# beecave-homelab/VibeVoice-ROCm

Measured on AMD Instinct MI355X. Metric: audio-sec/s, higher is better.
Workload: dtype bf16; 1 GPU; cfg2: VibeVoice-1.5B shapes, 1 speaker(s) x 203-frame voice prompt, 330-token prompt, 225 frames (30.0 s audio), CFG=2.0, 20 DPM-Solver++ steps, whole generate() incl. voice encode + prefill; global_batch=1, parallelism=replicas x1 (one dialogue per GPU), hipgraph=True

## Files before the change

### include/vv_hip.h

```cpp
#ifndef VV_HIP_H
#define VV_HIP_H

#include <stddef.h>
#include <stdint.h>

#ifdef __cplusplus
extern "C" {
#endif

typedef void* vv_stream_t;

enum { VV_F32 = 0, VV_BF16 = 1, VV_FP8 = 2  };
enum { VV_NF4 = 3 };
enum { VV_WQ_NF4 = 0x100 };
enum { VV_OK = 0, VV_E_ARG = -1, VV_E_HIP = -2, VV_E_UNSUPPORTED = -3 };
enum { VV_PRO_NONE = 0, VV_PRO_RMSNORM = 1, VV_PRO_SILU = 2 };
enum { VV_ACT_NONE = 0, VV_ACT_GELU = 1, VV_ACT_SWIGLU = 2 };
enum { VV_LIN_X_BF16 = 1, VV_LIN_OUT_BF16 = 2, VV_LIN_W_REUSED = 4, VV_LIN_W_FRAG = 8 };

const char* vv_last_error(void);
int vv_abi_version(void);
int vv_tune(const char* key, int value);
int vv_init(void);

// ... 185 lines not shown
int vv_encoder_forward(const vv_convnet* net, const float* wav, int64_t T, float* feat, void* ws, vv_stream_t stream);
int vv_convnet_reset(const vv_convnet* net, vv_stream_t stream);

typedef struct vv_connector { int wdt, din, hidden; const void* fc1; const float* b1; const float* norm_w; const void* fc2; const float* b2; } vv_connector;
int vv_connector_forward(const vv_connector* c, const float* x, int R, float* out, int accumulate, float* ws, vv_stream_t stream);
int vv_connector_pair(const vv_connector* ac, const vv_connector* sem, const float* latent, const float* semfeat, float* out, int64_t ldo,
                      int rows_out, float* ws, vv_stream_t stream);

int vv_graph_begin(vv_stream_t stream);
int vv_graph_end(vv_stream_t stream, void** graph_exec_out);
int vv_graph_launch(void* graph_exec, vv_stream_t stream);
int vv_graph_destroy(void* graph_exec);

typedef struct vv_prof_entry { int m, n, k, dual, wdt, count; double total_ms; } vv_prof_entry;
int vv_prof_begin(int max_records);
int vv_prof_end(vv_prof_entry* out, int max_out, int* n_out);

typedef struct vv_nf4_src {
  const uint8_t* packed;
  const void* absmax;
  const float* quant_map;
  const float* nested_absmax;
  const float* nested_map;
  float nested_offset;
  int nested_blocksize;
  int n, k, blocksize;
} vv_nf4_src;
int vv_nf4_import(const vv_nf4_src* src, void* w, int64_t ldw, int row0, int rows_total, void* cq, float* cs, vv_stream_t stream);

#define VV_CONV_HOT_GEMV 0
#define VV_CONV_HOT_ROW 1
typedef struct vv_conv_hot_shape { const char* name; int kind, m, n, k, bias, gate, res; } vv_conv_hot_shape;
int vv_conv_hot_shapes(vv_conv_hot_shape* out, int cap);

size_t vv_sizeof(const char* struct_name);

#ifdef __cplusplus
}
#endif
#endif
```

### vibevoice_rocm_amd/_lib.py

```python
from __future__ import annotations

import ctypes as C
import os

_HERE = os.path.dirname(os.path.abspath(__file__))
LIB_PATH = os.path.join(_HERE, "libvv_hip.so")

VV_F32, VV_BF16, VV_FP8, VV_NF4 = 0, 1, 2, 3
VV_WQ_NF4 = 0x100
PRO_NONE, PRO_RMSNORM, PRO_SILU = 0, 1, 2
ACT_NONE, ACT_GELU, ACT_SWIGLU = 0, 1, 2
LIN_X_BF16, LIN_OUT_BF16, LIN_W_REUSED, LIN_W_FRAG = 1, 2, 4, 8
VV_MAX_STAGES = 8
KVQ_DERIVE_SCALES = 1

vp = C.c_void_p
i64 = C.c_int64


class W8(C.Structure):
    _fields_ = [("q", vp), ("scale", vp)]


class LinArgs(C.Structure):
# ... 103 lines not shown
    "vv_add_rows_silu_bf16": (C.c_int, [vp, i64, vp, i64, vp, C.c_int, C.c_int, C.c_int, vp]),
    "vv_dpm_proj": (C.c_int, [vp, i64, C.c_float, C.POINTER(DpmCoef), vp, vp, vp, vp, vp, C.c_int, C.c_int, C.c_int, vp, i64, C.c_int, vp, vp]),
    "vv_embed_row": (C.c_int, [vp, C.c_int, i64, vp, vp, vp]),
    "vv_gather_rows": (C.c_int, [vp, C.c_int, i64, C.POINTER(C.c_int), C.c_int, vp, vp]),
    "vv_argmax_ids": (C.c_int, [vp, C.c_int, vp, vp, vp, vp]),
    "vv_cast_rows_bf16": (C.c_int, [vp, i64, C.c_int, C.c_int, C.c_int, vp, C.c_float, vp, i64, vp]),
    "vv_copy_rows": (C.c_int, [vp, i64, vp, i64, C.c_int, C.c_int, vp]),
    "vv_dpm_step": (C.c_int, [vp, i64, C.c_int, C.c_int, C.c_float, C.c_float, C.c_float, C.c_float, C.c_float,
                              C.c_float, C.c_int, vp, vp, vp]),
    "vv_advance_lens": (C.c_int, [vp, vp, C.c_int, C.c_int, vp, vp]),
    "vv_llm_ws_bytes": (C.c_size_t, [C.POINTER(Llm), C.c_int]),
    "vv_llm_forward": (C.c_int, [C.POINTER(Llm), C.POINTER(KV), vp, i64, C.c_int, vp, vp, vp, i64, vp, vp]),
    "vv_llm_tail": (C.c_int, [C.POINTER(Llm), vp, i64, C.c_int, vp, i64, vp, C.c_int, vp, vp, vp, vp, vp, C.c_int, C.c_int, vp, vp]),
    "vv_llm_tail_batch": (C.c_int, [C.POINTER(Llm), vp, i64, C.c_int, vp, i64, vp, C.c_int, vp, vp, vp, vp, vp, C.c_int, C.c_int, vp, vp, vp]),
    "vv_head_ws_bytes": (C.c_size_t, [C.POINTER(Head), C.c_int]),
    "vv_head_ws_bytes_batch": (C.c_size_t, [C.POINTER(Head), C.c_int, C.c_int]),
    "vv_head_sample_batch": (C.c_int, [C.POINTER(Head), vp, i64, vp, i64, vp, C.POINTER(DpmCoef), C.c_int, C.c_float, vp, i64, C.c_int, vp, vp]),
    "vv_head_ws_bytes_batch_sde": (C.c_size_t, [C.POINTER(Head), C.c_int, C.c_int]),
    "vv_head_sample_batch_sde": (C.c_int, [C.POINTER(Head), vp, i64, vp, i64, vp, C.POINTER(DpmCoef), C.c_int, C.c_float, vp, i64, C.c_int, vp, vp, i64, vp]),
    "vv_head_sample": (C.c_int, [C.POINTER(Head), vp, i64, vp, vp, C.POINTER(DpmCoef), C.c_int, C.c_float, vp, vp, vp, vp]),
    "vv_head_forward": (C.c_int, [C.POINTER(Head), vp, vp, vp, C.c_int, vp, vp, vp]),
    "vv_convnet_ws_bytes": (C.c_size_t, [C.POINTER(ConvNet), i64, C.c_int]),
    "vv_decoder_forward": (C.c_int, [C.POINTER(ConvNet), vp, C.c_int, C.c_float, C.c_float, vp, vp, vp]),
    "vv_encoder_forward": (C.c_int, [C.POINTER(ConvNet), vp, i64, vp, vp, vp]),
    "vv_convnet_reset": (C.c_int, [C.POINTER(ConvNet), vp]),
    "vv_connector_forward": (C.c_int, [C.POINTER(Connector), vp, C.c_int, vp, C.c_int, vp, vp]),
    "vv_connector_pair": (C.c_int, [C.POINTER(Connector), C.POINTER(Connector), vp, vp, vp, i64, C.c_int, vp, vp]),
    "vv_graph_begin": (C.c_int, [vp]),
    "vv_graph_end": (C.c_int, [vp, C.POINTER(vp)]),
    "vv_graph_launch": (C.c_int, [vp, vp]),
    "vv_graph_destroy": (C.c_int, [vp]),
    "vv_nf4_import": (C.c_int, [C.POINTER(Nf4Src), vp, i64, C.c_int, C.c_int, vp, vp, vp]),
    "vv_conv_hot_shapes": (C.c_int, [vp, C.c_int]),
    "vv_sizeof": (C.c_size_t, [C.c_char_p]),
    "vv_prof_begin": (C.c_int, [C.c_int]),
    "vv_prof_end": (C.c_int, [C.POINTER(ProfEntry), C.c_int, C.POINTER(C.c_int)]),
}


class VVError(RuntimeError):
    pass


_lib = None


def load():
    global _lib
    if _lib is not None:
        return _lib
    import torch
    if not os.path.exists(LIB_PATH):
        raise VVError(f"{LIB_PATH} is missing: build the HIP extension first (python -m vibevoice_rocm_amd.build). "
                      "The MI355X kernels are the only compute path of this package.")
    lib = C.CDLL(LIB_PATH)
    for name, (res, args) in PROTOTYPES.items():
        fn = getattr(lib, name)
        fn.restype = res
        fn.argtypes = args
    for cname, cls in _STRUCTS.items():
        n = lib.vv_sizeof(cname.encode())
        if n != C.sizeof(cls):
            raise VVError(f"ABI mismatch for {cname}: C side {n} bytes, ctypes mirror {C.sizeof(cls)} bytes")
    _lib = lib
    return lib

# ... 9 lines not shown
```

### vibevoice_rocm_amd/csrc/vv_common.h

```cpp
#ifndef VV_COMMON_H
#define VV_COMMON_H
#include <hip/hip_runtime.h>
#include <stdarg.h>
#include <stdint.h>
#include "vv_hip.h"

int vv_set_error(int code, const char* fmt, ...);

#define VV_CHECK_LAUNCH(name)                                                                    \
  do {                                                                                           \
    hipError_t e_ = hipGetLastError();                                                           \
    if (e_ != hipSuccess) return vv_set_error(VV_E_HIP, "%s: %s", name, hipGetErrorString(e_));  \
  } while (0)

#define VV_TRY(expr)            \
  do {                          \
    int rc_ = (expr);           \
    if (rc_) return rc_;        \
  } while (0)

struct vv_kv_args {
  void* k; void* v;
  int kvdt, layers, rows, kv_heads, s_max, head_dim;
  void* vt;
  vv_kv_args(const vv_kv& a) : k(a.k), v(a.v), kvdt(a.kvdt), layers(a.layers), rows(a.rows), kv_heads(a.kv_heads), s_max(a.s_max), head_dim(a.head_dim), vt(a.vt) {}
};
struct vv_kv_args8 : vv_kv_args {
  const float* kscale; const float* vscale;
  vv_kv_args8(const vv_kv& a) : vv_kv_args(a), kscale(a.kscale), vscale(a.vscale) {}
};

int vv_launch_gemv_stream(const vv_lin_args& a, hipStream_t s);
struct vv_gemv_hot_shape { const char* name; int m, n, k, dual, pro, mod, bias, gate, res, act, flags; };
extern "C" int vv_gemv_hot_shapes(vv_gemv_hot_shape* out, int cap);
int vv_launch_gemv_hot(const vv_lin_args& a, hipStream_t s);
void vv_gemv_hot_set(int mask);
int vv_launch_conv_hot_gemv(const vv_lin_args& a, hipStream_t s);
int vv_launch_conv_hot_row(const vv_block& B, const float* x, float* y, float* hidden, float* hist_new, int C, float eps, hipStream_t s);
void vv_conv_hot_set(int mask);
int vv_launch_gemv_rows(const vv_lin_args& a, float* part, size_t part_floats, int* tickets, size_t n_tickets, hipStream_t s);
size_t vv_gemv_rows_part_floats(int n, int dual);
size_t vv_gemv_rows_tickets(int n);
int vv_gemv_rows_init();
void vv_gemv_rows_set(int on, int blocks, int pers);
int vv_linear_ws(const vv_lin_args* a, const void* f1, const void* f2, float* part, size_t part_floats, int* tickets, size_t n_tickets,
                 vv_stream_t stream, const vv_w8* q1 = nullptr, const vv_w8* q2 = nullptr);
int vv_launch_mfma_gemm(const vv_lin_args& a, hipStream_t s);
int vv_mfma_gemm_init();
int vv_launch_attn_decode(const float* qkv, int64_t ld_qkv, int R, int heads, const vv_kv* kv, int layer, const float2* rope, const int* lens, float* out,
                          int64_t ldo, float* part, int* tickets, int nsplit, int part_cap, hipStream_t s);
int vv_attn_decode_ws(const float* qkv, int64_t ld_qkv, int R, int heads, const vv_kv* kv, int layer, const float* rope_table, const int* lens, float* out,
                      int64_t ldo, float* part, int* tickets, int nsplit, int part_cap, vv_stream_t stream);
int vv_launch_kv_quantize(const vv_kv* src, const vv_kv* dst, int src_row, int dst_row, int len, int flags, hipStream_t s);
int vv_launch_attn_prefill(const float* qkv, int64_t ld_qkv, int R, int heads, const vv_kv* kv, int layer, const int* lens, const int* cache_rows,
                           float* out, int64_t ldo, hipStream_t s);
int vv_head_init_fused(const vv_head* h, const float* noise, float* Xs, float* Ms, float* h0, int64_t ldh, hipStream_t s);
bool vv_head_boundary_supported(const vv_head* h);
int vv_head_boundary_fused(const vv_head* h, const float* hrows, int64_t ldh, const float* shift, const float* scale, int64_t ld_mod, float cfg,
                           const vv_dpm_coef* k, float* Xs, float* Ms, float* h_out, int64_t ldh_out, float* latent_out, hipStream_t s);
int vv_head_boundary_batch(const vv_head* h, const float* hrows, int64_t ldh, const float* shift, const float* scale, int64_t ld_mod, float cfg,
                           const vv_dpm_coef* k, float* Xs, float* Ms, int64_t state_stride, float* h_out, int64_t ldh_out, float* latent_out,
                           int64_t latent_stride, int B, hipStream_t s,
                           const float* nx = nullptr, int64_t nx_stride = 0);
int vv_head_sde_proj_fused(const vv_head* h, const float* sde_noise, int64_t ld_sde, int n_steps, int B, float* NX, hipStream_t s);
int vv_fused_init();
int vv_head_pre_fused(const vv_head* h, const float* cond2, int64_t ld_cond, const float* temb, int n_steps, void* c_bf16, const float* noise,
                      float* Xs, float* Ms, float* h0, int64_t ldh, hipStream_t s);
int vv_launch_connector_pair(const vv_connector* ac, const vv_connector* sem, const float* latent, const float* semfeat, float* out, int64_t ldo, int rows_out,
                             float* ws, hipStream_t s);
int vv_head_modulations_fused(const vv_head* h, const void* c_bf16, int rows, float* const* mod, float* modf, hipStream_t s);
struct vv_conv_ctx_item { float* pad; float* state; int ctx, T, C; const float* dw_w; float* hs; int affine; float scale, bias; };
// ... 59 lines not shown
```

### vibevoice_rocm_amd/csrc/vv_conv_hot.hip

```cpp
#include <hip/hip_runtime.h>
#include <hip/hip_bf16.h>
#include <stdint.h>

#include "vv_hip.h"
#include "vv_common.h"

namespace {

typedef unsigned short bf16_t;
typedef unsigned int u32x4 __attribute__((ext_vector_type(4)));
typedef float vf2 __attribute__((ext_vector_type(2)));
typedef __bf16 bf16x8 __attribute__((ext_vector_type(8)));
typedef float f32x16 __attribute__((ext_vector_type(16)));

__device__ __forceinline__ void unpack8(const u32x4 v, float (&o)[8]) {
  o[0] = __uint_as_float(v.x << 16); o[1] = __uint_as_float(v.x & 0xffff0000u);
  o[2] = __uint_as_float(v.y << 16); o[3] = __uint_as_float(v.y & 0xffff0000u);
  o[4] = __uint_as_float(v.z << 16); o[5] = __uint_as_float(v.z & 0xffff0000u);
  o[6] = __uint_as_float(v.w << 16); o[7] = __uint_as_float(v.w & 0xffff0000u);
}

template <bool NT>
__device__ __forceinline__ u32x4 ldw(const bf16_t* p) {
  const u32x4* q = reinterpret_cast<const u32x4*>(p);
  if constexpr (NT) return __builtin_nontemporal_load(q);
  else return *q;
}

__device__ __forceinline__ void fma_unit(const u32x4 wv, const float (&x)[8], vf2& p) {
  float w[8];
  unpack8(wv, w);
#pragma unroll
  for (int j = 0; j < 8; j += 2) p = __builtin_elementwise_fma(vf2{w[j], w[j + 1]}, vf2{x[j], x[j + 1]}, p);
}

__device__ __forceinline__ float gate_res(float v, float g, float r) {
#pragma clang fp contract(off)
  const float t = v * g;
  return t + r;
}

#define VV_FENCE4(v) asm volatile("" : "+v"((v).x), "+v"((v).y), "+v"((v).z), "+v"((v).w))

template <int N, int K, int NW, int R, bool GR>
__global__ __launch_bounds__(64 * NW) void conv_gemv_kernel(const vv_lin_args a) {
  constexpr int KU = K / (512 * NW);
// ... 163 lines not shown
      uint2 p;
      p.x = pack2(yv[j][0] * rstd2 * fw[j][0], yv[j][1] * rstd2 * fw[j][1]);
      p.y = pack2(yv[j][2] * rstd2 * fw[j][2], yv[j][3] * rstd2 * fw[j][3]);
      *reinterpret_cast<uint2*>(xh + c0[j]) = p;
      if (c0[j] >= ys0 && c0[j] < ys0 + C / ROW_WG) st4(y + c0[j], yv[j]);
    }
  }
  __syncthreads();
  f32x16 acc;
#pragma unroll
  for (int i = 0; i < 16; ++i) acc[i] = 0.f;
  {
    const bf16_t* xf = xh + wave * (C / 4) + hk;
#pragma unroll
    for (int s = 0; s < ST; ++s) {
      const u32x4 xb = *reinterpret_cast<const u32x4*>(xf + s * 16);
      acc = __builtin_amdgcn_mfma_f32_32x32x16_bf16(__builtin_bit_cast(bf16x8, wf[s]), __builtin_bit_cast(bf16x8, xb), acc, 0, 0, 0);
    }
  }
  if (lm == 0) {
#pragma unroll
    for (int r = 0; r < 16; ++r) red[(wave * 16 + r) * 2 + (lane >> 5)] = acc[r];
  }
  __syncthreads();
  if (tid < 32) {
    const int r = 4 * (tid >> 3) + (tid & 3), h = (tid >> 2) & 1;
    float s = 0.f;
#pragma unroll
    for (int w4 = 0; w4 < 4; ++w4) s += red[(w4 * 16 + r) * 2 + h];
    hidden[n0 + tid] = vv_gelu_as(s + b1v);
  }
}

#undef VV_FENCE4

constexpr int N_HOT = 4;
const vv_conv_hot_shape g_table[N_HOT] = {
    {"block.w2",         VV_CONV_HOT_GEMV, 1, 2048, 8192,  1,   1,   1},
    {"block.ffn_in_row", VV_CONV_HOT_ROW,  1, 8192, 2048,  1,   0,   0},
    {"dec.handover",     VV_CONV_HOT_GEMV, 1, 8192, 4096,  1,   0,   0},
    {"sem.handover",     VV_CONV_HOT_GEMV, 1, 2048, 16384, 1,   0,   0},
};

constexpr int HOT_DEFAULT = 0xf;
int g_hot = HOT_DEFAULT;

bool matches(const vv_conv_hot_shape& e, const vv_lin_args& a) {
  return e.kind == VV_CONV_HOT_GEMV && a.m == e.m && a.n == e.n && a.k == e.k && a.wdt == VV_BF16 && !a.w2 && a.pro == VV_PRO_NONE && !a.mod_scale &&
         !a.mod_shift && (a.bias != nullptr) == (e.bias != 0) && (a.gate != nullptr) == (e.gate != 0) && (!e.gate || a.gate_ld == 0) &&
         (a.res != nullptr) == (e.res != 0) && a.act == VV_ACT_NONE && a.flags == 0;
}

}

void vv_conv_hot_set(int mask) { g_hot = mask < 0 ? HOT_DEFAULT : mask; }

extern "C" int vv_conv_hot_shapes(vv_conv_hot_shape* out, int cap) {
  for (int i = 0; i < N_HOT && i < cap; ++i) out[i] = g_table[i];
  return N_HOT;
}

int vv_launch_conv_hot_gemv(const vv_lin_args& a, hipStream_t s) {
  if (!(g_hot & ((1 << N_HOT) - 1)) || a.m != 1 || a.wdt != VV_BF16) return 0;
  int id = -1;
  for (int i = 0; i < N_HOT; ++i)
    if ((g_hot >> i & 1) && matches(g_table[i], a)) { id = i; break; }
  const bool alt = (g_hot & 256) != 0;
  switch (id) {
    case 0:
      if (alt) hipLaunchKernelGGL((conv_gemv_kernel<2048, 8192, 4, 4, true>), dim3(512), dim3(256), 0, s, a);
      else hipLaunchKernelGGL((conv_gemv_kernel<2048, 8192, 4, 8, true>), dim3(256), dim3(256), 0, s, a);
      return 1;
    case 2:
      if (alt) hipLaunchKernelGGL((conv_gemv_kernel<8192, 4096, 4, 16, false>), dim3(512), dim3(256), 0, s, a);
      else hipLaunchKernelGGL((conv_gemv_kernel<8192, 4096, 4, 8, false>), dim3(1024), dim3(256), 0, s, a);
      return 1;
    case 3:
      if (alt) hipLaunchKernelGGL((conv_gemv_kernel<2048, 16384, 8, 8, false>), dim3(256), dim3(512), 0, s, a);
      else hipLaunchKernelGGL((conv_gemv_kernel<2048, 16384, 8, 4, false>), dim3(512), dim3(512), 0, s, a);
      return 1;
  }
  return 0;
}

int vv_launch_conv_hot_row(const vv_block& B, const float* x, float* y, float* hidden, float* hist_new, int C, float eps, hipStream_t s) {
  if (!(g_hot & 2) || C != ROW_C || !hist_new) return 0;
  if (!(g_hot & 512)) hipLaunchKernelGGL(row_in_kernel<false>, dim3(ROW_WG + 1), dim3(256), 0, s, x, y, hidden, hist_new, B, eps);
  else hipLaunchKernelGGL(row_in_kernel<true>, dim3(ROW_WG + 1), dim3(256), 0, s, x, y, hidden, hist_new, B, eps);
  return 1;
}
```

### vibevoice_rocm_amd/csrc/vv_convffn.hip

```cpp
#include <hip/hip_runtime.h>
#include <hip/hip_bf16.h>
#include <stdint.h>

#include "vv_hip.h"
#include "vv_common.h"

namespace {

typedef unsigned short bf16_t;
typedef __bf16 bf16x8 __attribute__((ext_vector_type(8)));
typedef float f32x16 __attribute__((ext_vector_type(16)));
typedef float f32x4 __attribute__((ext_vector_type(4)));
typedef unsigned int u32x4 __attribute__((ext_vector_type(4)));

#ifdef VV_CF_TIMING
__device__ unsigned long long g_cf_t[8];
#define CSTAMP(i) do { if (blockIdx.x == 0 && blockIdx.y == 0 && threadIdx.x == 0) { const long long t_ = wall_clock64(); g_cf_t[i] += (unsigned long long)(t_ - tprev_); tprev_ = t_; } } while (0)
#else
#define CSTAMP(i) do { } while (0)
#endif

constexpr int TR2 = 16;
constexpr int HALO = 6;

__device__ __forceinline__ unsigned int pack2(float a, float b) {
  const __hip_bfloat16 x = __float2bfloat16(a), y = __float2bfloat16(b);
  return (unsigned int)(*reinterpret_cast<const bf16_t*>(&x)) | ((unsigned int)(*reinterpret_cast<const bf16_t*>(&y)) << 16);
}
__device__ __forceinline__ float sq4(const float4 v) { return v.x * v.x + v.y * v.y + v.z * v.z + v.w * v.w; }

template <int C, int TRV, int NT = 256> struct InLay {
  static constexpr int VW = C >= 256 ? 4 : 2;
  static constexpr int F4 = C / 4;
  static constexpr int FV = C / VW;
  static constexpr int TPR = FV < NT ? FV : NT;
  static constexpr int NWV = NT / 64;
  static constexpr int CPT = FV / TPR;
  static constexpr int RP = NT / TPR;
  static constexpr int NI = (TRV + HALO + RP - 1) / RP;
  static constexpr int WR = NI * RP;
  static constexpr int WPR = TPR / 64;
  static constexpr int P1 = C + 8;
  static constexpr int ST = C / (16 * NWV);
  static constexpr size_t XN = (size_t)WR * C * 4;
  static constexpr size_t RED = (size_t)NWV * 16 * 64 * 4;
  static constexpr size_t XH = (size_t)(WR - HALO) * P1 * 2;
  static constexpr size_t PART = (size_t)2 * WR * 8 * 4;
  static constexpr size_t LDS = (XN > RED ? XN : RED) + XH + PART;
};

template <int VW> __device__ __forceinline__ void ldv(const float* p, float (&o)[VW]) {
  if constexpr (VW == 4) { const float4 t = *reinterpret_cast<const float4*>(p); o[0] = t.x; o[1] = t.y; o[2] = t.z; o[3] = t.w; }
// ... 301 lines not shown
  __syncthreads();
  f32x16 acc;
#pragma unroll
  for (int i = 0; i < 16; ++i) acc[i] = 0.f;
  {
    const bf16_t* xf = xh + wave * (C / 4) + hk;
#pragma unroll
    for (int s = 0; s < ST; ++s) {
      const u32x4 xb = *reinterpret_cast<const u32x4*>(xf + s * 16);
      acc = __builtin_amdgcn_mfma_f32_32x32x16_bf16(__builtin_bit_cast(bf16x8, wf[s]), __builtin_bit_cast(bf16x8, xb), acc, 0, 0, 0);
    }
  }
#pragma unroll
  for (int r = 0; r < 16; ++r) red[(wave * 16 + r) * 64 + lane] = acc[r];
  __syncthreads();
  if ((lane & 31) == 0) {
    float v[4];
#pragma unroll
    for (int i = 0; i < 4; ++i) {
      float s = 0.f;
#pragma unroll
      for (int w4 = 0; w4 < 4; ++w4) s += red[(w4 * 16 + 4 * eg + i) * 64 + lane];
      v[i] = s;
    }
    *reinterpret_cast<float4*>(hidden + n0 + 8 * eg + 4 * (lane >> 5)) =
        make_float4(vv_gelu_as(v[0] + b1v.x), vv_gelu_as(v[1] + b1v.y), vv_gelu_as(v[2] + b1v.z), vv_gelu_as(v[3] + b1v.w));
  }
}

template <int C, int NW>
__global__ __launch_bounds__(64 * NW) void ffn_out_kernel(const bf16_t* __restrict__ hidden, const float* res, float* out, const float* __restrict__ hist_new,
                                                          int T, const vv_block B) {
  constexpr int K = 4 * C, KW = K / NW, ST = KW / 32;
  __shared__ float red[NW * 4 * 64];
  const int tid = threadIdx.x, lane = tid & 63, wave = tid >> 6;
  const int n0 = blockIdx.x * 16, t0 = blockIdx.y * TR2;
  const int r16 = lane & 15, kq = lane >> 4;
  u32x4 wf[ST], hf[ST];
  {
    const bf16_t* wr = reinterpret_cast<const bf16_t*>(B.w2) + (int64_t)(n0 + r16) * K + wave * KW + 8 * kq;
    const bf16_t* hr = hidden + (int64_t)min(t0 + r16, T - 1) * K + wave * KW + 8 * kq;
#pragma unroll
    for (int s = 0; s < ST; ++s) {
      wf[s] = *reinterpret_cast<const u32x4*>(wr + s * 32);
      hf[s] = *reinterpret_cast<const u32x4*>(hr + s * 32);
    }
  }
  const int ei = (tid >> 6) & 3, el = tid & 63;
  const int en = n0 + 4 * (el >> 4) + ei, em = t0 + (el & 15);
  const bool ev = em < T && tid < 256;
  const float b2v = B.b2[en], fgv = B.ffn_gamma[en];
  const float rv = ev ? res[(int64_t)em * C + en] : 0.f;
  const bool mover = hist_new && B.hist && blockIdx.x == 0 && blockIdx.y == 0;
  constexpr int HN = (HALO * C / 4 + 64 * NW - 1) / (64 * NW);
  float4 hv[HN];
  if (mover) {
#pragma unroll
    for (int i = 0; i < HN; ++i) {
      const int e = tid + 64 * NW * i;
      hv[i] = e < HALO * C / 4 ? *reinterpret_cast<const float4*>(hist_new + 4 * (size_t)e) : make_float4(0.f, 0.f, 0.f, 0.f);
    }
  }
  f32x4 acc = {0.f, 0.f, 0.f, 0.f};
#pragma unroll
  for (int s = 0; s < ST; ++s)
    acc = __builtin_amdgcn_mfma_f32_16x16x32_bf16(__builtin_bit_cast(bf16x8, wf[s]), __builtin_bit_cast(bf16x8, hf[s]), acc, 0, 0, 0);
#pragma unroll
  for (int i = 0; i < 4; ++i) red[(wave * 4 + i) * 64 + lane] = acc[i];
  __syncthreads();
  if (ev) {
    float s = 0.f;
#pragma unroll
    for (int w4 = 0; w4 < NW; ++w4) s += red[(w4 * 4 + ei) * 64 + el];
    out[(int64_t)em * C + en] = rv + fgv * (s + b2v);
  }
  if (mover) {
#pragma unroll
    for (int i = 0; i < HN; ++i) {
      const int e = tid + 64 * NW * i;
      if (e < HALO * C / 4) *reinterpret_cast<float4*>(B.hist + 4 * (size_t)e) = hv[i];
    }
  }
}

template <int NST, int NB>
__global__ __launch_bounds__(256) void skinny_kernel(const float* __restrict__ x, int64_t ldx, int M, const bf16_t* __restrict__ W, int K,
                                                     const float* __restrict__ bias, float* __restrict__ out, int64_t ldo) {
  __shared__ float red[4 * 4 * 64];
  const int tid = threadIdx.x, lane = tid & 63, wave = tid >> 6;
  const int n0 = blockIdx.x * 16, t0 = blockIdx.y * 16;
  const int r16 = lane & 15, kq = lane >> 4;
  const int kb = wave * (32 * NST * NB) + 8 * kq;
  const bf16_t* wr = W + (int64_t)(n0 + r16) * K + kb;
  const float* xr = x + (int64_t)min(t0 + r16, M - 1) * ldx + kb;
  const int ei = tid >> 6, el = tid & 63;
  const int en = n0 + 4 * (el >> 4) + ei, em = t0 + (el & 15);
  const float bv = bias ? bias[en] : 0.f;
  f32x4 acc = {0.f, 0.f, 0.f, 0.f};
#pragma unroll
  for (int b = 0; b < NB; ++b) {
    u32x4 wf[NST];
    float4 xa[NST], xb[NST];
#pragma unroll
    for (int s = 0; s < NST; ++s) {
      wf[s] = *reinterpret_cast<const u32x4*>(wr + 32 * (b * NST + s));
      xa[s] = *reinterpret_cast<const float4*>(xr + 32 * (b * NST + s));
      xb[s] = *reinterpret_cast<const float4*>(xr + 32 * (b * NST + s) + 4);
    }
#pragma unroll
    for (int s = 0; s < NST; ++s) {
      u32x4 p;
      p.x = pack2(xa[s].x, xa[s].y); p.y = pack2(xa[s].z, xa[s].w); p.z = pack2(xb[s].x, xb[s].y); p.w = pack2(xb[s].z, xb[s].w);
      acc = __builtin_amdgcn_mfma_f32_16x16x32_bf16(__builtin_bit_cast(bf16x8, wf[s]), __builtin_bit_cast(bf16x8, p), acc, 0, 0, 0);
    }
  }
// ... 3 lines not shown
  if (em < M) {
    float v = 0.f;
#pragma unroll
    for (int w4 = 0; w4 < 4; ++w4) v += red[(w4 * 4 + ei) * 64 + el];
    out[(int64_t)em * ldo + en] = v + bv;
  }
}

int g_skinny = 1, g_skinny_min_m = 5, g_skinny_max_m = 2048;

int g_on = 1;

template <int C> constexpr int in_threads() { return (C == 512 || C == 1024) ? 512 : 256; }

template <int C, int TRV, int NW>
int launch_c(const vv_block& B, const float* x, float* y, void* hidden, float* hist_new, float* out, int T, float eps, hipStream_t s) {
  float* hn = B.hist ? hist_new : nullptr;
  constexpr int NT = in_threads<C>();
  constexpr size_t lds = InLay<C, TRV, NT>::LDS;
  hipLaunchKernelGGL((ffn_in_kernel<C, TRV, false, NT>), dim3(4 * C / 32, (T + TRV - 1) / TRV), dim3(NT), lds, s, x, y, hidden, hn, T, B, eps);
  hipLaunchKernelGGL((ffn_out_kernel<C, NW>), dim3(C / 16, (T + TR2 - 1) / TR2), dim3(64 * NW), 0, s, reinterpret_cast<const bf16_t*>(hidden), y, out, hn, T, B);
  return hipGetLastError() == hipSuccess ? 1 : vv_set_error(VV_E_HIP, "vv_convffn: launch failed");
}

int g_trv512 = 8, g_trv256 = 16, g_trv128 = 32;
int g_c128 = 1;

}

#ifdef VV_CF_TIMING
extern "C" int vv_convffn_debug_times(unsigned long long* out8, int reset) {
  if (hipMemcpyFromSymbol(out8, HIP_SYMBOL(g_cf_t), 8 * sizeof(unsigned long long)) != hipSuccess) return -1;
  if (reset) { unsigned long long z[8] = {0}; if (hipMemcpyToSymbol(HIP_SYMBOL(g_cf_t), z, sizeof(z)) != hipSuccess) return -1; }
  return 0;
}
#endif
void vv_convffn_set(int on) { g_on = on; }
void vv_convffn_set_rows(int c, int rows) { if (c == 512) g_trv512 = rows; else if (c == 256) g_trv256 = rows; else if (c == 128) g_trv128 = rows; }
void vv_convffn_set_c128(int on) { g_c128 = on; }
bool vv_convffn_prefers(int wdt, int T, int C) { return g_on && g_c128 && wdt == VV_BF16 && C == 128 && T >= 3 && T <= 1024; }
void vv_skinny_set(int on, int min_m, int max_m) { g_skinny = on; if (min_m > 0) g_skinny_min_m = min_m; if (max_m > 0) g_skinny_max_m = max_m; }

int vv_launch_skinny(const vv_lin_args& a, hipStream_t s) {
  if (!g_skinny || a.wdt != VV_BF16 || a.w2 || a.pro != VV_PRO_NONE || a.act != VV_ACT_NONE || a.gate || a.res || a.mod_scale || a.flags) return 0;
  if (a.m < g_skinny_min_m || a.m > g_skinny_max_m || a.n % 16 || a.ldx % 4 || a.ldx == 0 || ((uintptr_t)a.x % 16) || ((uintptr_t)a.w % 16)) return 0;
  dim3 grid(a.n / 16, (a.m + 15) / 16);
  const bf16_t* W = reinterpret_cast<const bf16_t*>(a.w);
#define VV_SK(NSTV, NBV) hipLaunchKernelGGL((skinny_kernel<NSTV, NBV>), grid, dim3(256), 0, s, a.x, a.ldx, a.m, W, a.k, a.bias, a.out, a.ldo)
  switch (a.k) {
    case 128: VV_SK(1, 1); break;
    case 256: VV_SK(2, 1); break;
    case 512: VV_SK(4, 1); break;
    case 1024: VV_SK(8, 1); break;
    case 2048: VV_SK(16, 1); break;
    case 2560: VV_SK(20, 1); break;
    case 5120: VV_SK(20, 2); break;
    default: return 0;
  }
#undef VV_SK
  return 1;
}

int vv_convffn_init() {
#define VV_CF_ATTR(CC, TT)                                                                                                                  \
  { constexpr int nt_ = in_threads<CC>(); constexpr int l_ = (int)InLay<CC, TT, nt_>::LDS;                                                 \
    if (hipFuncSetAttribute(reinterpret_cast<const void*>(&ffn_in_kernel<CC, TT, false, nt_>), hipFuncAttributeMaxDynamicSharedMemorySize, l_) != hipSuccess) \
      return vv_set_error(VV_E_HIP, "vv_convffn_init: cannot raise the LDS limit"); }
  VV_CF_ATTR(128, 16) VV_CF_ATTR(128, 32) VV_CF_ATTR(256, 8) VV_CF_ATTR(256, 16) VV_CF_ATTR(256, 32) VV_CF_ATTR(512, 8) VV_CF_ATTR(512, 16) VV_CF_ATTR(512, 32) VV_CF_ATTR(1024, 8)
#undef VV_CF_ATTR
  {
    constexpr int l1 = (int)InLay<2048, 1, 256>::LDS;
    if (hipFuncSetAttribute(reinterpret_cast<const void*>(&ffn_in_kernel<2048, 1, true, 256>), hipFuncAttributeMaxDynamicSharedMemorySize, l1) != hipSuccess)
      return vv_set_error(VV_E_HIP, "vv_convffn_init: cannot raise the LDS limit");
  }
  return 0;
}

int g_t1 = 1;
void vv_convffn_set_t1(int on) { g_t1 = on; }

int vv_launch_ffn_in_row(const vv_block& B, int wdt, const float* x, float* y, float* hidden, float* hist_new, int C, float eps, hipStream_t s) {
  if (!g_on || !g_t1 || wdt != VV_BF16 || C != 2048 || !B.hist) return 0;
  auto a16 = [](const void* q) { return q && ((uintptr_t)q % 16) == 0; };
  if (!a16(B.w1) || !a16(B.b1) || !a16(B.gamma) || !a16(B.norm_w) || !a16(B.ffn_norm_w) || !a16(B.dw_b) || !a16(B.dw_w) || !a16(x) || !a16(y) ||
      !a16(hidden) || !a16(hist_new) || !a16(B.hist) || x == y)
    return 0;
  constexpr size_t lds = InLay<2048, 1, 256>::LDS;
  hipLaunchKernelGGL((ffn_in_kernel<2048, 1, true, 256>), dim3(4 * 2048 / 32, 1), dim3(256), lds, s, x, y, hidden, hist_new, 1, B, eps);
  return hipGetLastError() == hipSuccess ? 1 : vv_set_error(VV_E_HIP, "vv_convffn: launch failed");
}

int g_t1hs = 1;
void vv_convffn_set_t1hs(int on) { g_t1hs = on; }

int vv_launch_ffn_in_row_hs(const vv_block& B, int wdt, const float* x, float* y, float* hidden, float* hist_new, int C, float eps, hipStream_t s) {
  if (!g_on || !g_t1 || !g_t1hs || wdt != VV_BF16 || C != 2048 || !B.hist || !B.hs || !B.dw_last) return 0;
  auto a16 = [](const void* q) { return q && ((uintptr_t)q % 16) == 0; };
  if (!a16(B.w1) || !a16(B.b1) || !a16(B.gamma) || !a16(B.norm_w) || !a16(B.ffn_norm_w) || !a16(B.dw_b) || !a16(B.dw_last) || !a16(B.hs) || !a16(x) ||
      !a16(y) || !a16(hidden) || !a16(hist_new) || !a16(B.hist) || x == y)
    return 0;
  if (!vv_launch_conv_hot_row(B, x, y, hidden, hist_new, C, eps, s))
    hipLaunchKernelGGL(ffn_in_row_kernel, dim3(4 * 2048 / 32), dim3(256), 0, s, x, y, hidden, hist_new, B, eps);
  return hipGetLastError() == hipSuccess ? 1 : vv_set_error(VV_E_HIP, "vv_convffn: launch failed");
}

int vv_launch_convffn(const vv_block& B, int wdt, const float* x, float* y, void* hidden, float* hist_new, float* out, int T, int C, float eps,
                      hipStream_t s) {
  if (!g_on || wdt != VV_BF16 || T < 3 || (C != 128 && C != 256 && C != 512 && C != 1024) || (C == 1024 && T > 64)) return 0;
  if (C == 128 ? (!g_c128 || T > 1024) : T > 256) return 0;
  auto a16 = [](const void* q) { return q && ((uintptr_t)q % 16) == 0; };
  if (!a16(B.w1) || !a16(B.w2) || !a16(B.b1) || !B.b2 || !a16(B.gamma) || !B.ffn_gamma || !a16(B.norm_w) || !a16(B.ffn_norm_w) || !a16(B.dw_b) ||
      !a16(B.dw_w) || !a16(x) || !a16(y) || !a16(hidden) || !a16(hist_new) || !out || (B.hist && !a16(B.hist)))
    return 0;
  {
    const uintptr_t xa = (uintptr_t)x, ya = (uintptr_t)y, bytes = (uintptr_t)T * C * 4;
    if (xa < ya + bytes && ya < xa + bytes) return 0;
  }
  if (C == 128) {
    if (g_trv128 == 16) return launch_c<128, 16, 4>(B, x, y, hidden, hist_new, out, T, eps, s);
    return launch_c<128, 32, 4>(B, x, y, hidden, hist_new, out, T, eps, s);
  }
  if (C == 256) {
    if (g_trv256 == 8) return launch_c<256, 8, 4>(B, x, y, hidden, hist_new, out, T, eps, s);
    if (g_trv256 == 16) return launch_c<256, 16, 4>(B, x, y, hidden, hist_new, out, T, eps, s);
    return launch_c<256, 32, 4>(B, x, y, hidden, hist_new, out, T, eps, s);
  }
  if (C == 512) {
    if (g_trv512 == 8) return launch_c<512, 8, 4>(B, x, y, hidden, hist_new, out, T, eps, s);
    if (g_trv512 == 16) return launch_c<512, 16, 4>(B, x, y, hidden, hist_new, out, T, eps, s);
    return launch_c<512, 32, 4>(B, x, y, hidden, hist_new, out, T, eps, s);
  }
  return launch_c<1024, 8, 8>(B, x, y, hidden, hist_new, out, T, eps, s);
}

extern "C" size_t vv_block_mid_ws_bytes(int T, int C) { return (size_t)T * C * 4 + (size_t)T * 4 * C * 2 + (size_t)HALO * C * 4 + 64; }

extern "C" int vv_block_mid(const vv_block* b, int wdt, const float* x, float* out, void* ws, int T, int C, float eps, vv_stream_t stream) {
  if (!b || !x || !out || !ws || T <= 0) return vv_set_error(VV_E_ARG, "vv_block_mid: bad args");
  float* y = reinterpret_cast<float*>(ws);
  char* hidden = reinterpret_cast<char*>(ws) + (size_t)T * C * 4;
  float* hn = reinterpret_cast<float*>(hidden + (size_t)T * 4 * C * 2);
  const int rc = vv_launch_convffn(*b, wdt, x, y, hidden, hn, out, T, C, eps, (hipStream_t)stream);
  if (rc < 0) return rc;
  if (rc == 0) return vv_set_error(VV_E_UNSUPPORTED, "vv_block_mid: shape not covered (C=%d T=%d wdt=%d)", C, T, wdt);
  return 0;
}
```

Before: 43.00 audio-sec/s.

## Add specialized C=1024 T=8 conv-block FFN in/out kernels with MFMA

```diff
diff --git a/include/vv_hip.h b/include/vv_hip.h
--- a/include/vv_hip.h
+++ b/include/vv_hip.h
@@ -241,6 +241,10 @@
 #define VV_CONV_HOT_ROW 1
 typedef struct vv_conv_hot_shape { const char* name; int kind, m, n, k, bias, gate, res; } vv_conv_hot_shape;
 int vv_conv_hot_shapes(vv_conv_hot_shape* out, int cap);
+#define VV_CONV_HOT_MID_IN 2
+#define VV_CONV_HOT_MID_OUT 3
+int vv_conv_hot_mid_shapes(vv_conv_hot_shape* out, int cap);
+int vv_conv_hot_mid_launches(int reset);
 
 size_t vv_sizeof(const char* struct_name);
 
diff --git a/vibevoice_rocm_amd/_lib.py b/vibevoice_rocm_amd/_lib.py
--- a/vibevoice_rocm_amd/_lib.py
+++ b/vibevoice_rocm_amd/_lib.py
@@ -159,6 +159,8 @@
     "vv_graph_destroy": (C.c_int, [vp]),
     "vv_nf4_import": (C.c_int, [C.POINTER(Nf4Src), vp, i64, C.c_int, C.c_int, vp, vp, vp]),
     "vv_conv_hot_shapes": (C.c_int, [vp, C.c_int]),
+    "vv_conv_hot_mid_shapes": (C.c_int, [vp, C.c_int]),
+    "vv_conv_hot_mid_launches": (C.c_int, [C.c_int]),
     "vv_sizeof": (C.c_size_t, [C.c_char_p]),
     "vv_prof_begin": (C.c_int, [C.c_int]),
     "vv_prof_end": (C.c_int, [C.POINTER(ProfEntry), C.c_int, C.POINTER(C.c_int)]),
diff --git a/vibevoice_rocm_amd/csrc/vv_common.h b/vibevoice_rocm_amd/csrc/vv_common.h
--- a/vibevoice_rocm_amd/csrc/vv_common.h
+++ b/vibevoice_rocm_amd/csrc/vv_common.h
@@ -37,6 +37,9 @@
 void vv_gemv_hot_set(int mask);
 int vv_launch_conv_hot_gemv(const vv_lin_args& a, hipStream_t s);
 int vv_launch_conv_hot_row(const vv_block& B, const float* x, float* y, float* hidden, float* hist_new, int C, float eps, hipStream_t s);
+int vv_launch_conv_hot_mid_in(const vv_block& B, const float* x, float* y, void* hidden, float* hist_new, int T, int C, float eps, hipStream_t s);
+int vv_launch_conv_hot_mid_out(const vv_block& B, const void* hidden, const float* res, float* out, const float* hist_new, int T, int C, hipStream_t s);
+int vv_conv_hot_init();
 void vv_conv_hot_set(int mask);
 int vv_launch_gemv_rows(const vv_lin_args& a, float* part, size_t part_floats, int* tickets, size_t n_tickets, hipStream_t s);
 size_t vv_gemv_rows_part_floats(int n, int dual);
diff --git a/vibevoice_rocm_amd/csrc/vv_conv_hot.hip b/vibevoice_rocm_amd/csrc/vv_conv_hot.hip
--- a/vibevoice_rocm_amd/csrc/vv_conv_hot.hip
+++ b/vibevoice_rocm_amd/csrc/vv_conv_hot.hip
@@ -12,6 +12,7 @@
 typedef float vf2 __attribute__((ext_vector_type(2)));
 typedef __bf16 bf16x8 __attribute__((ext_vector_type(8)));
 typedef float f32x16 __attribute__((ext_vector_type(16)));
+typedef float f32x4 __attribute__((ext_vector_type(4)));
 
 __device__ __forceinline__ void unpack8(const u32x4 v, float (&o)[8]) {
   o[0] = __uint_as_float(v.x << 16); o[1] = __uint_as_float(v.x & 0xffff0000u);
@@ -241,6 +242,229 @@
   }
 }
 
+constexpr int MID_C = 1024, MID_T = 8, MID_WR = 14, MID_P1 = MID_C + 8, MID_K = 4 * MID_C;
+constexpr size_t MID_XN = (size_t)MID_WR * MID_C * 4, MID_XH = (size_t)MID_T * MID_P1 * 2, MID_LDS = MID_XN + MID_XH + 2 * MID_WR * 8 * 4;
+
+template <int HC>
+__global__ __launch_bounds__(512) void mid_in_kernel(const float* __restrict__ x, float* __restrict__ y, bf16_t* __restrict__ hidden,
+                                                     float* __restrict__ hist_new, const vv_block B, float eps) {
+  constexpr int C = MID_C, P1 = MID_P1, NWG = 4 * C / HC, ST = C / (16 * 8);
+  extern __shared__ __attribute__((aligned(16))) unsigned char smem[];
+  float* xn = reinterpret_cast<float*>(smem);
+  float* red = reinterpret_cast<float*>(smem);
+  bf16_t* xh = reinterpret_cast<bf16_t*>(smem + MID_XN);
+  float* part = reinterpret_cast<float*>(smem + MID_XN + MID_XH);
+  float* part2 = part + MID_WR * 8;
+  const int tid = threadIdx.x, lane = tid & 63, wave = __builtin_amdgcn_readfirstlane(tid >> 6);
+  const int rloc = wave >> 2, slot = wave & 3;
+  const int c0 = 4 * (tid & 255);
+
+  if (blockIdx.x == NWG) {
+    float own[3][4], nw[4];
+#pragma unroll
+    for (int i = 0; i < 3; ++i) ld4(x + (size_t)(rloc + 2 * i + 2) * C + c0, own[i]);
+    ld4(B.norm_w + c0, nw);
+#pragma unroll
+    for (int i = 0; i < 3; ++i) {
+      float q = 0.f;
+#pragma unroll
+      for (int e = 0; e < 4; ++e) q = fmaf(own[i][e], own[i][e], q);
+      const float s = vv_wave_sum(q);
+      if (lane == 0) part[(rloc + 2 * i) * 8 + slot] = s;
+    }
+    __syncthreads();
+#pragma unroll
+    for (int i = 0; i < 3; ++i) {
+      const int j = rloc + 2 * i;
+      float ss = part[j * 8];
+#pragma unroll
+      for (int sl = 1; sl < 4; ++sl) ss += part[j * 8 + sl];
+      const float rstd = rsqrtf(ss / (float)C + eps);
+      float o[4];
+#pragma unroll
+      for (int e = 0; e < 4; ++e) o[e] = own[i][e] * rstd * nw[e];
+      st4(hist_new + (size_t)j * C + c0, o);
+    }
+    return;
+  }
+
+  const int n0 = blockIdx.x * HC;
+  const int lm = lane & 31, hk = (lane >> 5) * 8;
+  float own[7][4];
+  float nw[4], db[4], gm[4], fw[4], tap[28];
+#pragma unroll
+  for (int i = 3; i < 7; ++i) ld4(x + (size_t)(rloc + 2 * i - 6) * C + c0, own[i]);
+  ld4(B.norm_w + c0, nw);
+#pragma unroll
+  for (int i = 0; i < 3; ++i) ld4(B.hist + (size_t)(rloc + 2 * i) * C + c0, own[i]);
+  ld4(B.dw_b + c0, db);
+#pragma unroll
+  for (int q = 0; q < 7; ++q) {
+    float tq[4];
+    ld4(B.dw_w + (size_t)c0 * 7 + 4 * q, tq);
+#pragma unroll
+    for (int e = 0; e < 4; ++e) tap[4 * q + e] = tq[e];
+  }
+  ld4(B.gamma + c0, gm);
+  ld4(B.ffn_norm_w + c0, fw);
+  u32x4 wf[ST];
+  {
+    const bf16_t* wr = reinterpret_cast<const bf16_t*>(B.w1) + (size_t)(n0 + (lm & (HC - 1))) * C + wave * (C / 8) + hk;
+#pragma unroll
+    for (int s = 0; s < ST; ++s) wf[s] = ldw<false>(wr + s * 16);
+  }
+  const int em = tid & 7, eh = (tid >> 3) & 1, eg = (tid >> 4) & (HC / 8 - 1);
+  const float4 b1v = *reinterpret_cast<const float4*>(B.b1 + n0 + 8 * eg + 4 * eh);
+  __builtin_amdgcn_sched_barrier(0);
+
+#pragma unroll
+  for (int i = 3; i < 7; ++i) {
+    float q = 0.f;
+#pragma unroll
+    for (int e = 0; e < 4; ++e) q = fmaf(own[i][e], own[i][e], q);
+    const float s = vv_wave_sum(q);
+    if (lane == 0) part[(rloc + 2 * i) * 8 + slot] = s;
+  }
+#pragma unroll
+  for (int i = 0; i < 3; ++i) st4(xn + (rloc + 2 * i) * C + c0, own[i]);
+  __syncthreads();
+#pragma unroll
+  for (int i = 3; i < 7; ++i) {
+    const int w = rloc + 2 * i;
+    float ss = part[w * 8];
+#pragma unroll
+    for (int sl = 1; sl < 4; ++sl) ss += part[w * 8 + sl];
+    const float rstd = rsqrtf(ss / (float)C + eps);
+    float o[4];
+#pragma unroll
+    for (int e = 0; e < 4; ++e) o[e] = own[i][e] * rstd * nw[e];
+    st4(xn + w * C + c0, o);
+  }
+  __syncthreads();
+
+  float y1[4][4];
+#pragma unroll
+  for (int i = 3; i < 7; ++i) {
+    const int w = rloc + 2 * i, tt = w - 6;
+    float s[4];
+#pragma unroll
+    for (int e = 0; e < 4; ++e) s[e] = db[e];
+#pragma unroll
+    for (int k = 0; k < 7; ++k) {
+      float v[4];
+      ld4(xn + (tt + k) * C + c0, v);
+#pragma unroll
+      for (int e = 0; e < 4; ++e) s[e] = fmaf(tap[7 * e + k], v[e], s[e]);
+    }
+    float q = 0.f;
+#pragma unroll
+    for (int e = 0; e < 4; ++e) {
+      y1[i - 3][e] = own[i][e] + gm[e] * s[e];
+      q = fmaf(y1[i - 3][e], y1[i - 3][e], q);
+    }
+    const float s2 = vv_wave_sum(q);
+    if (lane == 0) part2[w * 8 + slot] = s2;
+  }
+  __syncthreads();
+  {
+    constexpr int YS = C / NWG;
+    const int ys0 = blockIdx.x * YS;
+#pragma unroll
+    for (int i = 3; i < 7; ++i) {
+      const int w = rloc + 2 * i, tt = w - 6;
+      float ss = part2[w * 8];
+#pragma unroll
+      for (int sl = 1; sl < 4; ++sl) ss += part2[w * 8 + sl];
+      const float rstd = rsqrtf(ss / (float)C + eps);
+      uint2 p;
+      p.x = pack2(y1[i - 3][0] * rstd * fw[0], y1[i - 3][1] * rstd * fw[1]);
+      p.y = pack2(y1[i - 3][2] * rstd * fw[2], y1[i - 3][3] * rstd * fw[3]);
+      *reinterpret_cast<uint2*>(xh + tt * P1 + c0) = p;
+      if (c0 >= ys0 && c0 < ys0 + YS) st4(y + (size_t)tt * C + c0, y1[i - 3]);
+    }
+  }
+  __syncthreads();
+
+  f32x16 acc;
+#pragma unroll
+  for (int i = 0; i < 16; ++i) acc[i] = 0.f;
+  {
+    const bf16_t* xf = xh + min(lm, MID_T - 1) * P1 + wave * (C / 8) + hk;
+#pragma unroll
+    for (int s = 0; s < ST; ++s) {
+      const u32x4 xb = *reinterpret_cast<const u32x4*>(xf + s * 16);
+      acc = __builtin_amdgcn_mfma_f32_32x32x16_bf16(__builtin_bit_cast(bf16x8, wf[s]), __builtin_bit_cast(bf16x8, xb), acc, 0, 0, 0);
+    }
+  }
+  if (lm < MID_T) {
+#pragma unroll
+    for (int r = 0; r < HC / 2; ++r) red[(wave * 16 + r) * 16 + (lane >> 5) * 8 + lm] = acc[r];
+  }
+  __syncthreads();
+  if (tid < 2 * HC) {
+    float v[4];
+#pragma unroll
+    for (int i = 0; i < 4; ++i) {
+      float s = 0.f;
+#pragma unroll
+      for (int w8 = 0; w8 < 8; ++w8) s += red[(w8 * 16 + 4 * eg + i) * 16 + eh * 8 + em];
+      v[i] = s;
+    }
+    uint2 p;
+    p.x = pack2(vv_gelu_as(v[0] + b1v.x), vv_gelu_as(v[1] + b1v.y));
+    p.y = pack2(vv_gelu_as(v[2] + b1v.z), vv_gelu_as(v[3] + b1v.w));
+    *reinterpret_cast<uint2*>(hidden + (size_t)em * MID_K + n0 + 8 * eg + 4 * eh) = p;
+  }
+}
+
+template <int CH>
+__global__ __launch_bounds__(512) void mid_out_kernel(const bf16_t* __restrict__ hidden, const float* res, float* out, const float* __restrict__ hist_new,
+                                                      const vv_block B) {
+  constexpr int C = MID_C, K = MID_K, KW = K / 8, ST = KW / 32, NWG = C / CH;
+  __shared__ float red[8 * 4 * 32];
+  const int tid = threadIdx.x, lane = tid & 63, wave = __builtin_amdgcn_readfirstlane(tid >> 6);
+  if (blockIdx.x == NWG) {
+    float4 hv[3];
+#pragma unroll
+    for (int i = 0; i < 3; ++i) hv[i] = *reinterpret_cast<const float4*>(hist_new + 4 * (size_t)(tid + 512 * i));
+#pragma unroll
+    for (int i = 0; i < 3; ++i) *reinterpret_cast<float4*>(B.hist + 4 * (size_t)(tid + 512 * i)) = hv[i];
+    return;
+  }
+  const int n0 = blockIdx.x * CH;
+  const int r16 = lane & 15, kq = lane >> 4;
+  u32x4 wf[ST], hf[ST];
+  {
+    const bf16_t* wr = reinterpret_cast<const bf16_t*>(B.w2) + (size_t)(n0 + (r16 & (CH - 1))) * K + wave * KW + 8 * kq;
+    const bf16_t* hr = hidden + (size_t)min(r16, MID_T - 1) * K + wave * KW + 8 * kq;
+#pragma unroll
+    for (int s = 0; s < ST; ++s) {
+      wf[s] = ldw<false>(wr + s * 32);
+      hf[s] = ldw<false>(hr + s * 32);
+    }
+  }
+  const int em = tid & 7, ec = (tid >> 3) & (CH - 1);
+  const int en = n0 + ec;
+  const float b2v = B.b2[en], fgv = B.ffn_gamma[en];
+  const float rv = res[(size_t)em * C + en];
+  __builtin_amdgcn_sched_barrier(0);
+  f32x4 acc = {0.f, 0.f, 0.f, 0.f};
+#pragma unroll
+  for (int s = 0; s < ST; ++s)
+    acc = __builtin_amdgcn_mfma_f32_16x16x32_bf16(__builtin_bit_cast(bf16x8, wf[s]), __builtin_bit_cast(bf16x8, hf[s]), acc, 0, 0, 0);
+  if (r16 < MID_T && kq < (CH + 3) / 4) {
+#pragma unroll
+    for (int i = 0; i < 4; ++i) red[(wave * 4 + i) * 32 + kq * 8 + r16] = acc[i];
+  }
+  __syncthreads();
+  if (tid < 8 * CH) {
+    float s = 0.f;
+#pragma unroll
+    for (int w8 = 0; w8 < 8; ++w8) s += red[(w8 * 4 + (ec & 3)) * 32 + (ec >> 2) * 8 + em];
+    out[(size_t)em * C + en] = fmaf(fgv, s + b2v, rv);
+  }
+}
+
 #undef VV_FENCE4
 
 constexpr int N_HOT = 4;
@@ -250,6 +474,13 @@
     {"dec.handover",     VV_CONV_HOT_GEMV, 1, 8192, 4096,  1,   0,   0},
     {"sem.handover",     VV_CONV_HOT_GEMV, 1, 2048, 16384, 1,   0,   0},
 };
+
+constexpr int N_MID = 2;
+const vv_conv_hot_shape g_mid_table[N_MID] = {
+    {"mid1024.ffn_in",   VV_CONV_HOT_MID_IN,  8, 4096, 1024, 1,   0,   0},
+    {"mid1024.ffn_out",  VV_CONV_HOT_MID_OUT, 8, 1024, 4096, 1,   1,   1},
+};
+constexpr int MID_IN_BIT = 1 << N_HOT, MID_OUT_BIT = 2 << N_HOT, MID_ALT = 1024;
 
 constexpr int HOT_DEFAULT = 0xf;
 int g_hot = HOT_DEFAULT;
@@ -298,3 +529,41 @@
   else hipLaunchKernelGGL(row_in_kernel<true>, dim3(ROW_WG + 1), dim3(256), 0, s, x, y, hidden, hist_new, B, eps);
   return 1;
 }
+
+int g_mid_launches = 0;
+
+extern "C" int vv_conv_hot_mid_launches(int reset) {
+  const int n = g_mid_launches;
+  if (reset) g_mid_launches = 0;
+  return n;
+}
+
+extern "C" int vv_conv_hot_mid_shapes(vv_conv_hot_shape* out, int cap) {
+  for (int i = 0; i < N_MID && i < cap; ++i) out[i] = g_mid_table[i];
+  return N_MID;
+}
+
+int vv_conv_hot_init() {
+  if (hipFuncSetAttribute(reinterpret_cast<const void*>(&mid_in_kernel<16>), hipFuncAttributeMaxDynamicSharedMemorySize, (int)MID_LDS) != hipSuccess ||
+      hipFuncSetAttribute(reinterpret_cast<const void*>(&mid_in_kernel<32>), hipFuncAttributeMaxDynamicSharedMemorySize, (int)MID_LDS) != hipSuccess)
+    return vv_set_error(VV_E_HIP, "vv_conv_hot_init: cannot raise the LDS limit");
+  return 0;
+}
+
+int vv_launch_conv_hot_mid_in(const vv_block& B, const float* x, float* y, void* hidden, float* hist_new, int T, int C, float eps, hipStream_t s) {
+  if (!(g_hot & MID_IN_BIT) || C != MID_C || T != MID_T || !B.hist || !hist_new || B.q_w1.q || B.q_w2.q) return 0;
+  ++g_mid_launches;
+  bf16_t* h = reinterpret_cast<bf16_t*>(hidden);
+  if (g_hot & MID_ALT) hipLaunchKernelGGL(mid_in_kernel<32>, dim3(4 * MID_C / 32 + 1), dim3(512), MID_LDS, s, x, y, h, hist_new, B, eps);
+  else hipLaunchKernelGGL(mid_in_kernel<16>, dim3(4 * MID_C / 16 + 1), dim3(512), MID_LDS, s, x, y, h, hist_new, B, eps);
+  return 1;
+}
+
+int vv_launch_conv_hot_mid_out(const vv_block& B, const void* hidden, const float* res, float* out, const float* hist_new, int T, int C, hipStream_t s) {
+  if (!(g_hot & MID_OUT_BIT) || C != MID_C || T != MID_T || !B.hist || !hist_new || B.q_w1.q || B.q_w2.q) return 0;
+  ++g_mid_launches;
+  const bf16_t* h = reinterpret_cast<const bf16_t*>(hidden);
+  if (g_hot & MID_ALT) hipLaunchKernelGGL(mid_out_kernel<8>, dim3(MID_C / 8 + 1), dim3(512), 0, s, h, res, out, hist_new, B);
+  else hipLaunchKernelGGL(mid_out_kernel<4>, dim3(MID_C / 4 + 1), dim3(512), 0, s, h, res, out, hist_new, B);
+  return 1;
+}
diff --git a/vibevoice_rocm_amd/csrc/vv_convffn.hip b/vibevoice_rocm_amd/csrc/vv_convffn.hip
--- a/vibevoice_rocm_amd/csrc/vv_convffn.hip
+++ b/vibevoice_rocm_amd/csrc/vv_convffn.hip
@@ -16,8 +16,11 @@
 #ifdef VV_CF_TIMING
 __device__ unsigned long long g_cf_t[8];
 #define CSTAMP(i) do { if (blockIdx.x == 0 && blockIdx.y == 0 && threadIdx.x == 0) { const long long t_ = wall_clock64(); g_cf_t[i] += (unsigned long long)(t_ - tprev_); tprev_ = t_; } } while (0)
+__device__ unsigned long long g_co_t[4];
+#define OSTAMP(i) do { if (blockIdx.x == 0 && blockIdx.y == 0 && threadIdx.x == 0) { const long long t_ = wall_clock64(); g_co_t[i] += (unsigned long long)(t_ - tprev_); tprev_ = t_; } } while (0)
 #else
 #define CSTAMP(i) do { } while (0)
+#define OSTAMP(i) do { } while (0)
 #endif
 
 constexpr int TR2 = 16;
@@ -385,6 +388,9 @@
 __global__ __launch_bounds__(64 * NW) void ffn_out_kernel(const bf16_t* __restrict__ hidden, const float* res, float* out, const float* __restrict__ hist_new,
                                                           int T, const vv_block B) {
   constexpr int K = 4 * C, KW = K / NW, ST = KW / 32;
+#ifdef VV_CF_TIMING
+  long long tprev_ = wall_clock64();
+#endif
   __shared__ float red[NW * 4 * 64];
   const int tid = threadIdx.x, lane = tid & 63, wave = tid >> 6;
   const int n0 = blockIdx.x * 16, t0 = blockIdx.y * TR2;
@@ -414,6 +420,7 @@
       hv[i] = e < HALO * C / 4 ? *reinterpret_cast<const float4*>(hist_new + 4 * (size_t)e) : make_float4(0.f, 0.f, 0.f, 0.f);
     }
   }
+  OSTAMP(0);
   f32x4 acc = {0.f, 0.f, 0.f, 0.f};
 #pragma unroll
   for (int s = 0; s < ST; ++s)
@@ -421,6 +428,7 @@
 #pragma unroll
   for (int i = 0; i < 4; ++i) red[(wave * 4 + i) * 64 + lane] = acc[i];
   __syncthreads();
+  OSTAMP(1);
   if (ev) {
     float s = 0.f;
 #pragma unroll
@@ -434,6 +442,7 @@
       if (e < HALO * C / 4) *reinterpret_cast<float4*>(B.hist + 4 * (size_t)e) = hv[i];
     }
   }
+  OSTAMP(2);
 }
 
 template <int NST, int NB>
@@ -503,6 +512,11 @@
 extern "C" int vv_convffn_debug_times(unsigned long long* out8, int reset) {
   if (hipMemcpyFromSymbol(out8, HIP_SYMBOL(g_cf_t), 8 * sizeof(unsigned long long)) != hipSuccess) return -1;
   if (reset) { unsigned long long z[8] = {0}; if (hipMemcpyToSymbol(HIP_SYMBOL(g_cf_t), z, sizeof(z)) != hipSuccess) return -1; }
+  return 0;
+}
+extern "C" int vv_convffn_out_debug_times(unsigned long long* out4, int reset) {
+  if (hipMemcpyFromSymbol(out4, HIP_SYMBOL(g_co_t), 4 * sizeof(unsigned long long)) != hipSuccess) return -1;
+  if (reset) { unsigned long long z[4] = {0}; if (hipMemcpyToSymbol(HIP_SYMBOL(g_co_t), z, sizeof(z)) != hipSuccess) return -1; }
   return 0;
 }
 #endif
@@ -539,6 +553,7 @@
       return vv_set_error(VV_E_HIP, "vv_convffn_init: cannot raise the LDS limit"); }
   VV_CF_ATTR(128, 16) VV_CF_ATTR(128, 32) VV_CF_ATTR(256, 8) VV_CF_ATTR(256, 16) VV_CF_ATTR(256, 32) VV_CF_ATTR(512, 8) VV_CF_ATTR(512, 16) VV_CF_ATTR(512, 32) VV_CF_ATTR(1024, 8)
 #undef VV_CF_ATTR
+  if (vv_conv_hot_init() != 0) return -1;
   {
     constexpr int l1 = (int)InLay<2048, 1, 256>::LDS;
     if (hipFuncSetAttribute(reinterpret_cast<const void*>(&ffn_in_kernel<2048, 1, true, 256>), hipFuncAttributeMaxDynamicSharedMemorySize, l1) != hipSuccess)
@@ -601,7 +616,15 @@
     if (g_trv512 == 16) return launch_c<512, 16, 4>(B, x, y, hidden, hist_new, out, T, eps, s);
     return launch_c<512, 32, 4>(B, x, y, hidden, hist_new, out, T, eps, s);
   }
-  return launch_c<1024, 8, 8>(B, x, y, hidden, hist_new, out, T, eps, s);
+  {
+    float* hn = B.hist ? hist_new : nullptr;
+    constexpr size_t lds_in = InLay<1024, 8, 512>::LDS;
+    const int hin = vv_launch_conv_hot_mid_in(B, x, y, hidden, hn, T, C, eps, s);
+    if (!hin) hipLaunchKernelGGL((ffn_in_kernel<1024, 8, false, 512>), dim3(128, (T + 7) / 8), dim3(512), lds_in, s, x, y, hidden, hn, T, B, eps);
+    if (!vv_launch_conv_hot_mid_out(B, hidden, y, out, hn, T, C, s))
+      hipLaunchKernelGGL((ffn_out_kernel<1024, 8>), dim3(64, (T + TR2 - 1) / TR2), dim3(512), 0, s, reinterpret_cast<const bf16_t*>(hidden), y, out, hn, T, B);
+    return hipGetLastError() == hipSuccess ? 1 : vv_set_error(VV_E_HIP, "vv_convffn: launch failed");
+  }
 }
 
 extern "C" size_t vv_block_mid_ws_bytes(int T, int C) { return (size_t)T * C * 4 + (size_t)T * 4 * C * 2 + (size_t)HALO * C * 4 + 64; }
```

Measured after the change: 42.91 audio-sec/s. No clear change (-0.2%).
